# tsai0507/PolishPathPlanning

Hardware: NVIDIA B200
Metric: points/sec kNN(k=16)+normals+slicing (higher is better)
Workload: dtype f32

## Files before the change

polishpathplanning_b200/csrc/api.cu:

```cuda
#include <stdarg.h>
#include <string.h>

#include <algorithm>
#include <cmath>
#include <string>
#include <vector>

#include "ppp_internal.cuh"
#include <cstring>
#include <cuda.h>

static thread_local char g_err[1024] = "";

void ppp_set_error(const char* fmt, ...) {
  va_list ap;
  va_start(ap, fmt);
  vsnprintf(g_err, sizeof(g_err), fmt, ap);
  va_end(ap);
}

#define LOCK(ctx) ApiScope _api_scope(ctx)

#define REQUIRE(cond, msg)            \
  do {                                \
    if (!(cond)) {                    \
      ppp_set_error("%s: %s", __func__, msg); \
      return PPP_ERR_INVALID;         \
    }                                 \
  } while (0)

extern "C" {

int ppp_abi_version(void) { return PPP_ABI_VERSION; }
const char* ppp_last_error(void) { return g_err; }

int ppp_create(int device, ppp_ctx** out) {
  if (!out) { ppp_set_error("ppp_create: out is NULL"); return PPP_ERR_INVALID; }
  *out = nullptr;
  int ndev = 0;
  cudaError_t e = cudaGetDeviceCount(&ndev);
  if (e != cudaSuccess || ndev == 0) {
    ppp_set_error("ppp_create: no CUDA device (%s); libppp_gpu has no CPU fallback",
                  e != cudaSuccess ? cudaGetErrorString(e) : "device count 0");
    cudaGetLastError();
    return PPP_ERR_CUDA;
  }
  if (device < 0 || device >= ndev) { ppp_set_error("ppp_create: device %d out of range [0,%d)", device, ndev); return PPP_ERR_INVALID; }
  PPP_CUDA(cudaSetDevice(device));
  cudaDeviceProp prop;
  PPP_CUDA(cudaGetDeviceProperties(&prop, device));
  if (prop.major < 10) {
    ppp_set_error("ppp_create: device %d is sm_%d%d; this library is built for sm_100a (B200) only", device, prop.major, prop.minor);
    return PPP_ERR_UNSUPPORTED;
  }
  ppp_ctx* ctx = new ppp_ctx();
  ctx->device = device;
  ctx->sm_count = prop.multiProcessorCount;
  ctx->smem_optin = prop.sharedMemPerBlockOptin;
  int prio_lo = 0, prio_hi = 0;
  PPP_CUDA(cudaDeviceGetStreamPriorityRange(&prio_lo, &prio_hi));
  PPP_CUDA(cudaStreamCreateWithPriority(&ctx->main_stream, cudaStreamNonBlocking, prio_lo));
  PPP_CUDA(cudaStreamCreateWithPriority(&ctx->aux_stream, cudaStreamNonBlocking, prio_hi));
  PPP_CUDA(cudaStreamCreateWithFlags(&ctx->copy_stream, cudaStreamNonBlocking));
  PPP_CUDA(cudaHostAlloc(&ctx->fetch_host, FETCH_BYTES + 128, cudaHostAllocMapped));
  *fetch_flag(ctx) = 0u;
  ctx->stream = ctx->main_stream;
  cudaMemPool_t pool;
  PPP_CUDA(cudaDeviceGetDefaultMemPool(&pool, device));
  uint64_t thr = UINT64_MAX;
  PPP_CUDA(cudaMemPoolSetAttribute(pool, cudaMemPoolAttrReleaseThreshold, &thr));
  *out = ctx;
  return PPP_OK;
}

void ppp_destroy(ppp_ctx* ctx) {
  if (!ctx) return;
  cudaSetDevice(ctx->device);
  cudaStreamSynchronize(ctx->main_stream);
  cudaStreamSynchronize(ctx->aux_stream);
  for (auto& kv : ctx->kstats)
    for (auto& p : kv.second.pending) { cudaEventDestroy(p.first); cudaEventDestroy(p.second); }
  for (int t = 0; t < 16; t++)
    for (auto& p : ctx->t_pending[t]) { cudaEventDestroy(p.first); cudaEventDestroy(p.second); }
  cudaStreamDestroy(ctx->main_stream);
  if (ctx->aux_stream) cudaStreamDestroy(ctx->aux_stream);
  if (ctx->copy_stream) cudaStreamDestroy(ctx->copy_stream);
  if (ctx->fetch_host) cudaFreeHost(ctx->fetch_host);
  for (int i = 0; i < 2; i++) if (ctx->scan_state[i]) cudaFree(ctx->scan_state[i]);
  if (ctx->ingest_dev) cudaFree(ctx->ingest_dev);
  delete ctx;
}

void* ppp_stream(ppp_ctx* ctx) { return ctx ? (void*)ctx->main_stream : nullptr; }

int ppp_sync(ppp_ctx* ctx) {
  REQUIRE(ctx, "ctx is NULL");
  PPP_CUDA(cudaStreamSynchronize(ctx->main_stream));
  return PPP_OK;
}

void* ppp_host_alloc(size_t bytes) {
  void* p = nullptr;
  if (cudaMallocHost(&p, bytes ? bytes : 1) != cudaSuccess) { cudaGetLastError(); return nullptr; }
  return p;
}
void ppp_host_free(void* p) { if (p) cudaFreeHost(p); }

int64_t ppp_launch_count(ppp_ctx* ctx) { return ctx ? ctx->launches : 0; }

int ppp_timer_begin(ppp_ctx* ctx, int tag) {
  REQUIRE(ctx && tag >= 0 && tag < 16, "bad ctx/tag");
  LOCK(ctx);
  cudaEvent_t a, b;
  PPP_CUDA(cudaEventCreate(&a));
  PPP_CUDA(cudaEventCreate(&b));
  PPP_CUDA(cudaEventRecord(a, ctx->main_stream));
  ctx->t_pending[tag].emplace_back(a, b);
  return PPP_OK;
}
int ppp_timer_end(ppp_ctx* ctx, int tag) {
  REQUIRE(ctx && tag >= 0 && tag < 16, "bad ctx/tag");
  LOCK(ctx);
  REQUIRE(!ctx->t_pending[tag].empty(), "timer_end without timer_begin");
  PPP_CUDA(cudaEventRecord(ctx->t_pending[tag].back().second, ctx->main_stream));
  return PPP_OK;
}
int ppp_timer_read(ppp_ctx* ctx, int tag, double* total_ms, int64_t* regions, int reset) {
  REQUIRE(ctx && tag >= 0 && tag < 16, "bad ctx/tag");
  LOCK(ctx);
  PPP_CUDA(cudaStreamSynchronize(ctx->main_stream));
  for (auto& p : ctx->t_pending[tag]) {
    float ms = 0;
    PPP_CUDA(cudaEventElapsedTime(&ms, p.first, p.second));
    ctx->t_ms[tag] += ms;
    ctx->t_regions[tag]++;
    cudaEventDestroy(p.first);
    cudaEventDestroy(p.second);
  }
  ctx->t_pending[tag].clear();
  if (total_ms) *total_ms = ctx->t_ms[tag];
  if (regions) *regions = ctx->t_regions[tag];
  if (reset) { ctx->t_ms[tag] = 0; ctx->t_regions[tag] = 0; }
  return PPP_OK;
}

int ppp_kernel_profile(ppp_ctx* ctx, int enable) {
  REQUIRE(ctx, "ctx is NULL");
  LOCK(ctx);
  ctx->profile = enable != 0;
  return PPP_OK;
}
int ppp_kernel_profile_read(ppp_ctx* ctx, char* buf, size_t cap, int reset) {
  REQUIRE(ctx && buf && cap > 0, "bad arguments");
  LOCK(ctx);
  PPP_CUDA(cudaStreamSynchronize(ctx->main_stream));
  PPP_CUDA(cudaStreamSynchronize(ctx->aux_stream));
  std::string s;
  for (auto& kv : ctx->kstats) {
    KernelStat& st = kv.second;
    for (auto& p : st.pending) {
      float ms = 0;
      if (cudaEventElapsedTime(&ms, p.first, p.second) == cudaSuccess) { st.ms += ms; st.launches++; }
      cudaEventDestroy(p.first);
      cudaEventDestroy(p.second);
    }
    st.pending.clear();
    char line[256];
    snprintf(line, sizeof(line), "%s=%.6f:%lld;", kv.first.c_str(), st.ms, (long long)st.launches);
    s += line;
  }
  if (reset) ctx->kstats.clear();
// ... 794 lines not shown
```

polishpathplanning_b200/csrc/grid.cu:

```cuda
#include <stdlib.h>

#include <algorithm>
#include <cmath>

#include "ppp_device.cuh"

namespace {

__device__ __forceinline__ uint32_t f2ord(float f) {
  uint32_t b = __float_as_uint(f);
  return (b & 0x80000000u) ? ~b : (b | 0x80000000u);
}
inline float ord2f(uint32_t u) {
  uint32_t b = (u & 0x80000000u) ? (u & 0x7FFFFFFFu) : ~u;
  float f;
  memcpy(&f, &b, 4);
  return f;
}

__host__ __device__ inline int ds_sub_shift(long long n) {
  int sh = 0;
  while ((n >> sh) >= 16384) sh++;
  return sh;
}
// ... 37 lines not shown
          x[j] = p.x; y[j] = p.y; z[j] = p.z;
        } else {
          const float* p = raw + i * sf;
          x[j] = __ldg(p); y[j] = __ldg(p + 1); z[j] = __ldg(p + 2);
        }
      }
    }
#pragma unroll
    for (int j = 0; j < PPT; j++) {
      int64_t i = base + (int64_t)j * blockDim.x + threadIdx.x;
      if (i >= n) continue;
      bool fin = finite3(x[j], y[j], z[j]);
      const float4 rec = make_float4(x[j], y[j], z[j], fin ? 0.0f : CUDART_NAN_F);
      xyz4[i] = rec;
      PPP_DEV_ASSERT(!sub || (i >> sub_shift) < 16384);
      if (sub && (i & sub_mask) == 0) sub[i >> sub_shift] = rec;
      if (fin) {
        cnt++;
        mn[0] = fminf(mn[0], x[j]); mx[0] = fmaxf(mx[0], x[j]);
        mn[1] = fminf(mn[1], y[j]); mx[1] = fmaxf(mx[1], y[j]);
        mn[2] = fminf(mn[2], z[j]); mx[2] = fmaxf(mx[2], z[j]);
      }
    }
  }
#pragma unroll
  for (int o = 16; o > 0; o >>= 1) {
#pragma unroll
    for (int d = 0; d < 3; d++) {
      mn[d] = fminf(mn[d], __shfl_xor_sync(0xffffffffu, mn[d], o));
      mx[d] = fmaxf(mx[d], __shfl_xor_sync(0xffffffffu, mx[d], o));
    }
    cnt += __shfl_xor_sync(0xffffffffu, cnt, o);
  }
  __shared__ float s_mn[8][3], s_mx[8][3];
  __shared__ unsigned s_cnt[8];
  const int w = threadIdx.x >> 5;
  if ((threadIdx.x & 31) == 0) {
#pragma unroll
    for (int d = 0; d < 3; d++) { s_mn[w][d] = mn[d]; s_mx[w][d] = mx[d]; }
    s_cnt[w] = cnt;
  }
  __syncthreads();
  if (threadIdx.x == 0) {
    unsigned tot = 0;
    for (int i = 0; i < (int)(blockDim.x >> 5); i++) {
      tot += s_cnt[i];
#pragma unroll
      for (int d = 0; d < 3; d++) { mn[d] = fminf(mn[d], s_mn[i][d]); mx[d] = fmaxf(mx[d], s_mx[i][d]); }
    }
    if (tot) {
#pragma unroll
      for (int d = 0; d < 3; d++) {
        atomicMin(&acc->mn[d], f2ord(mn[d]));
        atomicMax(&acc->mx[d], f2ord(mx[d]));
      }
      atomicAdd(&acc->n_finite, (unsigned long long)tot);
    }
  }
}

__device__ __forceinline__ int cell_of(const GridView& g, float x, float y, float z) {
  int cu = clampi(cell_coord_raw(axis_of(x, y, z, g.au), g.min_u, g.inv_h), 0, g.nu - 1);
  int cv = clampi(cell_coord_raw(axis_of(x, y, z, g.av), g.min_v, g.inv_h), 0, g.nv - 1);
  return cv * g.nu + cu;
}

__global__ void __launch_bounds__(256) k_cell_count(GridView g, const float4* __restrict__ xyz4, int64_t n,
                                                    int32_t* __restrict__ counts) {
  pdl_prologue();
  int64_t i = (int64_t)blockIdx.x * blockDim.x + threadIdx.x;
  if (i >= n) return;
  float4 p = __ldg(xyz4 + i);
  if (p.w != p.w) return;
  const int cell = cell_of(g, p.x, p.y, p.z);
  PPP_DEV_ASSERT(cell >= 0 && cell < g.nu * g.nv);
  atomicAdd(counts + cell, 1);
}

__global__ void __launch_bounds__(256) k_cell_scatter(GridView g, const float4* __restrict__ xyz4, int64_t n,
                                                      int32_t* __restrict__ counts, const int32_t* __restrict__ start,
                                                      float4* __restrict__ sorted) {
  pdl_prologue();
  int64_t i = (int64_t)blockIdx.x * blockDim.x + threadIdx.x;
  if (i >= n) return;
  float4 p = __ldg(xyz4 + i);
  if (p.w != p.w) return;
  int c = cell_of(g, p.x, p.y, p.z);
  int slot = __ldg(start + c) + atomicSub(counts + c, 1) - 1;
  PPP_DEV_ASSERT(c >= 0 && c < g.nu * g.nv && slot >= 0 && slot < g.n_sorted);
  sorted[slot] = make_float4(p.x, p.y, p.z, __int_as_float((int)i));
}

__global__ void __launch_bounds__(256) k_extract_order(const float4* __restrict__ sorted, int64_t n, int32_t* __restrict__ order) {
  pdl_prologue();
  int64_t i = (int64_t)blockIdx.x * blockDim.x + threadIdx.x;
  if (i < n) order[i] = __float_as_int(__ldg(&sorted[i].w));
}

constexpr int DS_KTH = 8;
constexpr int DS_THREADS = 512;
__device__ __forceinline__ float ds_ord2f(uint32_t u) {
  uint32_t b = (u & 0x80000000u) ? (u & 0x7FFFFFFFu) : ~u;
  return __uint_as_float(b);
}

__device__ __forceinline__ float ds_kth_smallest(const float* s) {
  float v[2 * DS_THREADS / 32];
#pragma unroll
  for (int i = 0; i < 2 * DS_THREADS / 32; i++) v[i] = s[i * 32 + (threadIdx.x & 31)];
  float kth = CUDART_INF_F;
  for (int r = 0; r < DS_KTH; r++) {
    float mine = CUDART_INF_F;
    int at = 0;
#pragma unroll
    for (int i = 0; i < 2 * DS_THREADS / 32; i++) if (v[i] < mine) { mine = v[i]; at = i; }
    float w = mine;
#pragma unroll
    for (int o = 16; o > 0; o >>= 1) w = fminf(w, __shfl_xor_sync(0xffffffffu, w, o));
    kth = w;
    const unsigned holders = __ballot_sync(0xffffffffu, mine == w && w < CUDART_INF_F);
    if (holders && (int)(threadIdx.x & 31) == __ffs(holders) - 1) {
#pragma unroll
      for (int i = 0; i < 2 * DS_THREADS / 32; i++) if (i == at) v[i] = CUDART_INF_F;
    }
  }
  return kth;
}

struct IngestScratch {
  BBoxAcc acc;
  unsigned ticket;
  unsigned pad[3];
  float samples[2 * 128];
};

__global__ void __launch_bounds__(DS_THREADS) k_density_sample(const float4* __restrict__ xyz4, int64_t n, int64_t stride_s,
                                                               const float4* __restrict__ sub, int m, IngestScratch* __restrict__ scr, int S,
                                                               unsigned* __restrict__ host_out, unsigned* __restrict__ host_flag,
                                                               unsigned seq, const long long* __restrict__ n_dev,
                                                               const unsigned* __restrict__ extra_src, int extra_words) {
  pdl_prologue();
  __shared__ float s_d[2 * DS_THREADS], s_p[2 * DS_THREADS];
  __shared__ bool s_last;
  if (n_dev) {
    n = *n_dev;
    const long long ds_s = n < (long long)gridDim.x ? n : (long long)gridDim.x;
    stride_s = ds_s > 0 ? (n / ds_s > 1 ? n / ds_s : 1) : 1;
    const int sh = ds_sub_shift(n);
    m = (int)((n + ((long long)1 << sh) - 1) >> sh);
  }
  const BBoxAcc* acc = &scr->acc;
  float* out = scr->samples;
  int drop = 2;
  {
    double ext[3];
    for (int d = 0; d < 3; d++) ext[d] = (double)ds_ord2f(acc->mx[d]) - (double)ds_ord2f(acc->mn[d]);
    if (ext[1] < ext[drop]) drop = 1;
    if (ext[0] < ext[drop]) drop = 0;
  }
  const bool has_q = (int64_t)blockIdx.x * stride_s < n;
  const float4 q = has_q ? __ldg(xyz4 + (int64_t)blockIdx.x * stride_s) : make_float4(0.f, 0.f, 0.f, CUDART_NAN_F);
  const bool qfin = q.w == q.w;
  float d0 = CUDART_INF_F, d1 = CUDART_INF_F, p0 = CUDART_INF_F, p1 = CUDART_INF_F;
  if (qfin) {
    constexpr int PPT = 8;
    for (int j0 = (int)threadIdx.x; j0 < m; j0 += DS_THREADS * PPT) {
// ... 151 lines not shown
  for (int d = 0; d < 3; d++) {
    c->bmin[d] = c->n_finite ? ord2f(h.mn[d]) : 3.402823466e+38f;
    c->bmax[d] = c->n_finite ? ord2f(h.mx[d]) : -3.402823466e+38f;
  }
  double ext[3];
  for (int d = 0; d < 3; d++) ext[d] = c->n_finite ? (double)c->bmax[d] - (double)c->bmin[d] : 0.0;
  int drop = 2;
  if (ext[1] < ext[drop]) drop = 1;
  if (ext[0] < ext[drop]) drop = 0;
  c->drop = drop;
  c->au = drop == 0 ? 1 : 0;
  c->av = drop == 2 ? 1 : 2;
  double area = std::max(ext[c->au], 1e-9) * std::max(ext[c->av], 1e-9);
  c->density = c->n_finite > 0 ? (double)c->n_finite / area : 0.0;
  std::vector<float> r2;
  int piled = 0;
  for (int i = 0; i < ds_s; i++)
    if (std::isfinite(ds_h[i]) && ds_h[i] > 0) {
      r2.push_back(ds_h[i]);
      piled += ds_h[DS_SAMPLES + i] * 4.0f < ds_h[i] ? 1 : 0;
    }
  c->mp_state = (r2.size() >= 32 && c->n_finite >= 4096 && piled * 25 > (int)r2.size()) ? 1 : 0;
  if (const char* e = getenv("PPP_PROJECTIONS")) {
    if (e[0] == '1') c->mp_state = 0;
    if (e[0] == '3') c->mp_state = 1;
  }
  if (getenv("PPP_DEBUG"))
    fprintf(stderr, "[ppp] ingest: %d of %zu samples pile up in projection -> %s\n", piled, r2.size(),
            c->mp_state ? "three projections" : "one column grid");
  if (r2.size() >= 16 && c->n_finite >= 64) {
    std::nth_element(r2.begin(), r2.begin() + r2.size() / 2, r2.end());
    const double r2_med = (double)r2[r2.size() / 2];
    const double seen = (double)((c->n + stride_m - 1) / stride_m) * ((double)c->n_finite / (double)c->n);
    const double rho_sub = 7.67 / (3.14159265358979 * r2_med);
    c->density = rho_sub * (double)c->n_finite / std::max(seen, 1.0);
  }
  return PPP_OK;
}

double cloud_cell_for_k(const ppp_cloud* c, int k) {
  if (c->cell_hint > 0) return c->cell_hint;
  double rho = c->density > 0 ? c->density : 1.0;
  double rk = std::sqrt((double)std::max(k, 1) / (3.14159265358979 * rho));
  double f = 1.35;
  if (const char* e = getenv("PPP_CELL_FACTOR")) { double v = atof(e); if (v > 0.5 && v < 4.0) f = v; }
  return f * rk / (double)PPP_KNN_RINGS;
}
double cloud_cell_for_radius(const ppp_cloud* c, double r) {
  (void)c;
  return r * 0.5 * (1.0 + 1e-3);
}

int cloud_get_grid(ppp_cloud* c, double h, GridStore** out) { return cloud_get_grid_drop(c, h, c->drop, out); }

int cloud_get_grid_drop(ppp_cloud* c, double h, int drop, GridStore** out) {
  ppp_ctx* ctx = c->ctx;
  const int au = drop == 0 ? 1 : 0, av = drop == 2 ? 1 : 2;
  double eu = c->n_finite ? (double)c->bmax[au] - (double)c->bmin[au] : 0.0;
  double ev = c->n_finite ? (double)c->bmax[av] - (double)c->bmin[av] : 0.0;
  if (!(h > 0)) h = 1.0;
  while ((std::floor(eu / h) + 2) * (std::floor(ev / h) + 2) > 268435456.0) h *= 1.5;
  for (auto& g : c->grids)
    if (g.drop == drop && std::fabs(g.h - h) <= 1e-9 * h) { *out = &g; return PPP_OK; }
  if (c->grids.size() >= c->grids.capacity()) {
    ppp_set_error("too many different cell sizes on one cloud (%zu grids)", c->grids.size());
    return PPP_ERR_UNSUPPORTED;
  }
  GridStore gs;
  gs.h = h;
  gs.drop = drop;
  GridView& v = gs.v;
  v.au = au; v.av = av;
  v.h = (float)h;
  v.inv_h = 1.0f / v.h;
  v.min_u = c->n_finite ? c->bmin[au] : 0.0f;
  v.min_v = c->n_finite ? c->bmin[av] : 0.0f;
  v.nu = (int)std::floor(eu * (double)v.inv_h) + 2;
  v.nv = (int)std::floor(ev * (double)v.inv_h) + 2;
  v.slack = (float)(h * (double)(v.nu + v.nv) * 9.5367431640625e-07 + 1e-30);
  v.n_sorted = (int)c->n_finite;
  int64_t ncells = (int64_t)v.nu * v.nv;
  PPP_TRY(dev_alloc_keep(ctx, &gs.sorted, (size_t)std::max<int64_t>(c->n_finite, 1) + PPP_SORTED_PAD));
  PPP_TRY(dev_alloc_keep(ctx, &gs.cell_start, (size_t)ncells + 1));
  int32_t* counts = nullptr;
  PPP_TRY(dev_alloc(ctx, &counts, (size_t)ncells));
  PPP_CUDA(cudaMemsetAsync(counts, 0, (size_t)ncells * sizeof(int32_t), ctx->stream));
  v.sorted = gs.sorted;
  v.cell_start = gs.cell_start;
  if (c->n > 0) {
    unsigned blocks = (unsigned)((c->n + 255) / 256);
    PPP_LAUNCH(ctx, "cell_count", k_cell_count, blocks, 256, 0, v, (const float4*)c->xyz4, c->n, counts);
    PPP_CHECK_LAUNCH();
  }
  PPP_TRY(scan_exclusive_i32(ctx, counts, gs.cell_start, ncells));
  if (c->n > 0) {
    unsigned blocks = (unsigned)((c->n + 255) / 256);
    PPP_LAUNCH(ctx, "cell_scatter", k_cell_scatter, blocks, 256, 0, v, (const float4*)c->xyz4, c->n, counts,
               (const int32_t*)gs.cell_start, gs.sorted);
    PPP_CHECK_LAUNCH();
  }
  dev_free(ctx, counts);
  PPP_CUDA(cudaEventCreateWithFlags(&gs.ready, cudaEventDisableTiming));
  PPP_CUDA(cudaEventRecord(gs.ready, ctx->stream));
  c->grids.push_back(gs);
  *out = &c->grids.back();
  return PPP_OK;
}

int cloud_decide_projection(ppp_cloud* c, const GridStore& g) {
  (void)g;
  if (c->mp_state < 0) c->mp_state = 0;
  return PPP_OK;
}

int cloud_get_mp(ppp_cloud* c, double h, int R0, MPSet** out) {
  ppp_ctx* ctx = c->ctx;
  for (auto& m : c->mps)
    if (m.R0 == R0 && std::fabs(m.h - h) <= 1e-9 * h) { *out = &m; return PPP_OK; }
  if (c->mps.size() >= c->mps.capacity()) { ppp_set_error("too many multi-projection index sets on one cloud"); return PPP_ERR_UNSUPPORTED; }
  MPSet m;
  m.h = h; m.R0 = R0;
  for (int p = 0; p < 3; p++) PPP_TRY(cloud_get_grid_drop(c, h, p, &m.g[p]));
  PPP_TRY(dev_alloc_keep(ctx, &m.choice, (size_t)std::max<int64_t>(c->n, 1)));
  unsigned long long* hist = nullptr;
  PPP_TRY(dev_alloc(ctx, &hist, 3));
  PPP_CUDA(cudaMemsetAsync(hist, 0, 3 * sizeof(unsigned long long), ctx->stream));
  if (c->n > 0) {
    G3 G;
    for (int p = 0; p < 3; p++) G.g[p] = m.g[p]->v;
    PPP_LAUNCH(ctx, "mp_choose", k_mp_choose, (unsigned)((c->n + 255) / 256), 256, 0, G, (const float4*)c->xyz4, c->n, R0,
               m.choice, hist);
    PPP_CHECK_LAUNCH();
  }
  if (getenv("PPP_DEBUG")) {
    unsigned long long hh[3] = {0, 0, 0};
    PPP_TRY(fetch_small(ctx, hist, sizeof(hh), hh));
    fprintf(stderr, "[ppp] projections chosen (h = %g, R0 = %d): yz %llu, xz %llu, xy %llu\n", h, R0, hh[0], hh[1], hh[2]);
  }
  dev_free(ctx, hist);
  PPP_CUDA(cudaEventCreateWithFlags(&m.ready, cudaEventDisableTiming));
  PPP_CUDA(cudaEventRecord(m.ready, ctx->stream));
  c->mps.push_back(m);
  *out = &c->mps.back();
  return PPP_OK;
}

int grid_sorted_order(ppp_cloud* c, GridStore& gs) {
  if (gs.order) return PPP_OK;
  ppp_ctx* ctx = c->ctx;
  const int64_t n = gs.v.n_sorted;
  PPP_TRY(dev_alloc_keep(ctx, &gs.order, (size_t)std::max<int64_t>(n, 1)));
  if (n > 0) {
    PPP_LAUNCH(ctx, "extract_order", k_extract_order, (unsigned)((n + 255) / 256), 256, 0, (const float4*)gs.sorted, n, gs.order);
    PPP_CHECK_LAUNCH();
  }
  return PPP_OK;
}

__global__ void k_fetch_small(const unsigned* __restrict__ src, unsigned* __restrict__ dst, int words,
                              unsigned* __restrict__ flag, unsigned seq) {
  pdl_prologue();
  for (int i = threadIdx.x; i < words; i += blockDim.x) dst[i] = src[i];
  __threadfence_system();
  __syncthreads();
  if (threadIdx.x == 0) *(volatile unsigned*)flag = seq;
}

int fetch_wait(ppp_ctx* ctx, unsigned seq) {
  volatile unsigned* flag = fetch_flag(ctx);
  for (unsigned long spin = 1;; spin++) {
    if (*flag == seq) return PPP_OK;
    if ((spin & 0x1FFFul) == 0) {
      cudaError_t e = cudaStreamQuery(ctx->stream);
      if (e == cudaSuccess) {
        if (*flag == seq) return PPP_OK;
        ppp_set_error("fetch: the stream drained without the kernel signalling (sequence %u)", seq);
        return PPP_ERR_CUDA;
      }
      if (e != cudaErrorNotReady) {
        ppp_set_error("fetch: %s", cudaGetErrorString(e));
        return PPP_ERR_CUDA;
      }
    }
  }
// ... 18 lines not shown
```

polishpathplanning_b200/csrc/knn.cu:

```cuda
#include <stdlib.h>

#include <algorithm>
#include <cmath>

#include "ppp_device.cuh"
#include "sortnet.cuh"

namespace {

struct SearchParams {
  GridView g;
  const float4* xyz4;
  const float* q;
  int q_sf;
  int64_t nq;
  int64_t first;
  int cap;
  int kk;
  int mode;
  int R0;
  float r2;
  int32_t* idx_out;
  float* d2_out;
  const int64_t* offsets;
// ... 596 lines not shown
      int a = max(cu - R, 0), b = min(cu + R, g.nu - 1);
      if (a <= b) {
        const int32_t* rowp = g.cell_start + (int64_t)v * g.nu;
        s = __ldg(rowp + a);
        e = __ldg(rowp + b + 1);
      }
    }
    const int n_it = (__reduce_max_sync(0xffffffffu, e - s) + U - 1) / U;
#pragma unroll 1
    for (int it = 0; it < n_it; it++) {
      float4 c4[U];
      bool in[U];
#pragma unroll
      for (int u = 0; u < U; u++) {
        int i = s + it * U + u;
        in[u] = i < e;
        c4[u] = __ldg(g.sorted + (in[u] ? i : 0));
      }
      u64* wptr = store + ns * BD;
#pragma unroll
      for (int u = 0; u < U; u++) {
        float d2 = d2_flann_x2(pack2(qx, qy), qz, c4[u]);
        u64 key = make_key(d2, __float_as_int(c4[u].w));
        if (in[u] && key < tau) {
          *wptr = key;
          wptr += BD;
        }
      }
      ns = (int)(wptr - store) / BD;
      if (ns > C_STORE - U) { overflow = true; tau = 0; }
    }
  }
  if (!valid) return;
  unsigned c[C_SLOTS];
#pragma unroll
  for (int i = 0; i < C_SLOTS; i++) {
    unsigned hi = (unsigned)(store[i * BD] >> 32);
    c[i] = i < ns ? ((hi & 0xFFFFFFE0u) | (unsigned)i) : 0xFFFFFFFFu;
  }
  SortNetU32<C_SLOTS>::sort(c);
  bool ambiguous = false;
#pragma unroll
  for (int i = 0; i + 1 < C_SLOTS; i++) ambiguous |= (i + 1 < ns) && ((c[i] ^ c[i + 1]) < 32u);
  if (overflow || ns > C_SLOTS || ambiguous) {
    int slot = atomicAdd(P.redo_count, 1);
    P.redo_list[slot] = (int32_t)t;
    return;
  }
  float o[4];
  const int m = ns;
  if (!act || m < 3) {
    o[0] = o[1] = o[2] = o[3] = CUDART_NAN_F;
  } else {
    float acc[9] = {0.f, 0.f, 0.f, 0.f, 0.f, 0.f, 0.f, 0.f, 0.f};
    const bool shifted = (P.flags & PPP_COV_SHIFTED) != 0;
    float kx = 0.f, ky = 0.f, kz = 0.f;
    if (shifted) {
      float4 f = __ldg(P.xyz4 + key_idx(store[(c[0] & 31u) * BD]));
      kx = f.x; ky = f.y; kz = f.z;
    }
#pragma unroll
    for (int jb = 0; jb < C_SLOTS; jb += 4) {
      if (jb < m) {
        float4 a[4];
#pragma unroll
        for (int u = 0; u < 4; u++)
          if (jb + u < m) a[u] = __ldg(P.xyz4 + key_idx(store[(c[jb + u] & 31u) * BD]));
#pragma unroll
        for (int u = 0; u < 4; u++) {
          if (jb + u < m) {
            float x = a[u].x, y = a[u].y, z = a[u].z;
            if (shifted) { x = __fsub_rn(x, kx); y = __fsub_rn(y, ky); z = __fsub_rn(z, kz); }
            accumulate_point(acc, x, y, z);
          }
        }
      }
    }
    normal_from_accumulators(acc, m, qx, qy, qz, P.vpx, P.vpy, P.vpz, o);
  }
  store_normal(P.normals, P.nmap, row, P.nsf, o, P.route);
}

__device__ __forceinline__ u64 warp_min_u64(u64 v) {
#pragma unroll
  for (int o = 16; o > 0; o >>= 1) {
    u64 t = __shfl_xor_sync(0xffffffffu, v, o);
    v = t < v ? t : v;
  }
  return v;
}

constexpr int WARPQ_WARPS = 4;

constexpr int WQ_SEG_MAX = 128;

__global__ void __launch_bounds__(WARPQ_WARPS * 32) k_knn_warp(SearchParams P) {
  pdl_prologue();
  extern __shared__ u64 s_keys[];
  __shared__ int s_seg[WARPQ_WARPS][WQ_SEG_MAX];
  __shared__ int s_pre[WARPQ_WARPS][WQ_SEG_MAX + 1];
  const int lane = threadIdx.x & 31, w = threadIdx.x >> 5;
  const GridView& g = P.g;
  const int k = P.cap, kk = P.kk;
  u64* L = s_keys + (size_t)w * 32 * k + lane;
  const int n_redo = *P.redo_count;
  for (int64_t slot = (int64_t)blockIdx.x * WARPQ_WARPS + w; slot < n_redo; slot += (int64_t)gridDim.x * WARPQ_WARPS) {
  const int64_t t = P.redo_list[slot];
  float qx, qy, qz;
  int64_t row;
  if (P.q) {
    const float* qp = P.q + t * P.q_sf;
    qx = __ldg(qp); qy = __ldg(qp + 1); qz = __ldg(qp + 2);
    row = t;
  } else {
    float4 p = __ldg(g.sorted + P.first + t);
    qx = p.x; qy = p.y; qz = p.z;
    row = __float_as_int(p.w);
  }
  const int cu = cell_coord_raw(axis_of(qx, qy, qz, g.au), g.min_u, g.inv_h);
  const int cv = cell_coord_raw(axis_of(qx, qy, qz, g.av), g.min_v, g.inv_h);
  int cnt = 0;
  u64 tau = PPP_KEY_INF;
  u64 mine = PPP_KEY_INF;
  u64 mine2 = PPP_KEY_INF;
  int du = max(max(-cu, cu - (g.nu - 1)), 0), dv0 = max(max(-cv, cv - (g.nv - 1)), 0);
  int R = max(P.R0, max(du, dv0));
  int R_prev = -1;
  while (true) {
    const int v0 = max(cv - R, 0), v1 = min(cv + R, g.nv - 1);
    const int nseg = 2 * (v1 - v0 + 1);
    if (nseg > 0 && nseg <= WQ_SEG_MAX) {
      int* seg_s = s_seg[w];
      int* seg_p = s_pre[w];
      for (int sg0 = 0; sg0 < nseg; sg0 += 32) {
        const int sg = sg0 + lane;
        int s0 = 0, len = 0;
        if (sg < nseg) {
          const int v = v0 + (sg >> 1), part = sg & 1;
          const bool full = abs(v - cv) > R_prev;
          int a, b;
          if (full) { a = max(cu - R, 0); b = part == 0 ? min(cu + R, g.nu - 1) : -1; }
          else if (part == 0) { a = max(cu - R, 0); b = min(cu - R_prev - 1, g.nu - 1); }
          else { a = max(cu + R_prev + 1, 0); b = min(cu + R, g.nu - 1); }
          if (a <= b) {
            const int32_t* rowp = g.cell_start + (int64_t)v * g.nu;
            s0 = __ldg(rowp + a);
            len = __ldg(rowp + b + 1) - s0;
          }
        }
        int inc = len;
#pragma unroll
        for (int o = 1; o < 32; o <<= 1) { int tt = __shfl_up_sync(0xffffffffu, inc, o); if (lane >= o) inc += tt; }
        const int carry = sg0 == 0 ? 0 : seg_p[sg0];
        if (sg < nseg) { seg_s[sg] = s0; seg_p[sg + 1] = carry + inc; }
        if (sg0 == 0 && lane == 0) seg_p[0] = 0;
        __syncwarp();
      }
      const int T = seg_p[nseg];
      for (int base = 0; base < T; base += 128) {
        float4 c4[4];
        bool in[4];
#pragma unroll
        for (int u = 0; u < 4; u++) {
          const int i = base + u * 32 + lane;
          in[u] = i < T;
          int lo = 0, hi = nseg - 1;
          while (lo < hi) { int mid = (lo + hi + 1) >> 1; if (seg_p[mid] <= i) lo = mid; else hi = mid - 1; }
          c4[u] = __ldg(g.sorted + (in[u] ? seg_s[lo] + (i - seg_p[lo]) : 0));
        }
#pragma unroll
        for (int u = 0; u < 4; u++) {
          if (!in[u]) continue;
          u64 key = make_key(d2_flann(qx, qy, qz, c4[u].x, c4[u].y, c4[u].z), __float_as_int(c4[u].w));
          if (key < tau && (cnt < k || key < L[(k - 1) * 32])) list_insert(L, 32, cnt, k, key);
        }
      }
    } else {
    for (int v = v0; v <= v1; v++) {
      const int32_t* rowp = g.cell_start + (int64_t)v * g.nu;
      const bool full = abs(v - cv) > R_prev;
      for (int part = 0; part < (full ? 1 : 2); part++) {
        int a, b;
        if (full) { a = max(cu - R, 0); b = min(cu + R, g.nu - 1); }
        else if (part == 0) { a = max(cu - R, 0); b = min(cu - R_prev - 1, g.nu - 1); }
        else { a = max(cu + R_prev + 1, 0); b = min(cu + R, g.nu - 1); }
        if (a > b) continue;
        const int s = __ldg(rowp + a), e = __ldg(rowp + b + 1);
        for (int i = s + lane; i < e; i += 32) {
          float4 c = __ldg(g.sorted + i);
          u64 key = make_key(d2_flann(qx, qy, qz, c.x, c.y, c.z), __float_as_int(c.w));
          if (key < tau && (cnt < k || key < L[(k - 1) * 32])) list_insert(L, 32, cnt, k, key);
        }
      }
    }
    }
    __syncwarp();
    int head = 0;
    u64 kth = PPP_KEY_INF;
    mine = PPP_KEY_INF;
    mine2 = PPP_KEY_INF;
    for (int j = 0; j < kk; j++) {
      u64 h = head < cnt ? L[head * 32] : PPP_KEY_INF;
      u64 m = warp_min_u64(h);
      if (m == PPP_KEY_INF) break;
      if (h == m) head++;
      if (lane == (j & 31)) { if (j < 32) mine = m; else mine2 = m; }
      kth = (j == kk - 1) ? m : kth;
    }
    if (kth != PPP_KEY_INF && key_d2(kth) < ring_bound2(g, R, cu, cv)) break;
    if (block_covers_grid(g, cu, cv, R)) break;
    if (kth != PPP_KEY_INF) tau = kth;
    R_prev = R;
    R++;
  }
  const int have = __popc(__ballot_sync(0xffffffffu, mine != PPP_KEY_INF)) +
                   __popc(__ballot_sync(0xffffffffu, mine2 != PPP_KEY_INF));
  if (P.idx_out && lane < k) {
    P.idx_out[row * (int64_t)k + lane] = mine != PPP_KEY_INF ? key_idx(mine) : -1;
    if (P.d2_out) P.d2_out[row * (int64_t)k + lane] = mine != PPP_KEY_INF ? key_d2(mine) : CUDART_INF_F;
  }
  if (P.idx_out && 32 + lane < k) {
    P.idx_out[row * (int64_t)k + 32 + lane] = mine2 != PPP_KEY_INF ? key_idx(mine2) : -1;
    if (P.d2_out) P.d2_out[row * (int64_t)k + 32 + lane] = mine2 != PPP_KEY_INF ? key_d2(mine2) : CUDART_INF_F;
  }
  if (P.normals) {
    float o[4];
    if (have < 3) {
      o[0] = o[1] = o[2] = o[3] = CUDART_NAN_F;
    } else {
      float acc[9] = {0.f, 0.f, 0.f, 0.f, 0.f, 0.f, 0.f, 0.f, 0.f};
      const bool shifted = (P.flags & PPP_COV_SHIFTED) != 0;
      float kx = 0.f, ky = 0.f, kz = 0.f;
      float4 rec = make_float4(0.f, 0.f, 0.f, 0.f), rec2 = rec;
      if (mine != PPP_KEY_INF) rec = __ldg(P.xyz4 + key_idx(mine));
      if (mine2 != PPP_KEY_INF) rec2 = __ldg(P.xyz4 + key_idx(mine2));
      for (int j = 0; j < have; j++) {
        const bool lo32 = j < 32;
        float4 a;
        a.x = __shfl_sync(0xffffffffu, lo32 ? rec.x : rec2.x, j & 31);
        a.y = __shfl_sync(0xffffffffu, lo32 ? rec.y : rec2.y, j & 31);
        a.z = __shfl_sync(0xffffffffu, lo32 ? rec.z : rec2.z, j & 31);
        if (shifted && j == 0) { kx = a.x; ky = a.y; kz = a.z; }
        float x = a.x, y = a.y, z = a.z;
        if (shifted) { x = __fsub_rn(x, kx); y = __fsub_rn(y, ky); z = __fsub_rn(z, kz); }
        accumulate_point(acc, x, y, z);
      }
      normal_from_accumulators(acc, have, qx, qy, qz, P.vpx, P.vpy, P.vpz, o);
    }
    if (lane == 0) store_normal(P.normals, P.nmap, row, P.nsf, o, P.route);
  }
  __syncwarp();
  }
}

constexpr int RW_CAPL = 16;

__global__ void __launch_bounds__(WARPQ_WARPS * 32) k_radius_warp(SearchParams P, int32_t* __restrict__ redo2_count,
                                                                  int32_t* __restrict__ redo2_list) {
  pdl_prologue();
  __shared__ u64 s_l[WARPQ_WARPS * 32 * RW_CAPL];
  const int lane = threadIdx.x & 31, w = threadIdx.x >> 5;
  const GridView& g = P.g;
  u64* L = s_l + (size_t)w * 32 * RW_CAPL + lane;
  const int n_redo = *P.redo_count;
  const u64 tau = make_key(P.r2, 0);
  for (int64_t slot = (int64_t)blockIdx.x * WARPQ_WARPS + w; slot < n_redo; slot += (int64_t)gridDim.x * WARPQ_WARPS) {
    const int64_t t = P.redo_list[slot];
    float4 p = __ldg(g.sorted + P.first + t);
    const float qx = p.x, qy = p.y, qz = p.z;
    const int64_t row = __float_as_int(p.w);
    const int cu = cell_coord_raw(axis_of(qx, qy, qz, g.au), g.min_u, g.inv_h);
    const int cv = cell_coord_raw(axis_of(qx, qy, qz, g.av), g.min_v, g.inv_h);
    const int R = P.R0;
    int cnt = 0;
    bool over = false;
    const int v0 = max(cv - R, 0), v1 = min(cv + R, g.nv - 1);
    for (int v = v0; v <= v1; v++) {
      const int32_t* rowp = g.cell_start + (int64_t)v * g.nu;
      int a = max(cu - R, 0), b = min(cu + R, g.nu - 1);
      if (a > b) continue;
      const int s = __ldg(rowp + a), e = __ldg(rowp + b + 1);
      for (int i = s + lane; i < e; i += 32) {
        float4 c = __ldg(g.sorted + i);
        u64 key = make_key(d2_flann(qx, qy, qz, c.x, c.y, c.z), __float_as_int(c.w));
        if (key < tau) {
          if (cnt == RW_CAPL) over = true;
          else list_insert(L, 32, cnt, RW_CAPL, key);
        }
      }
    }
    __syncwarp();
    if (__any_sync(0xffffffffu, over)) {
      if (lane == 0) redo2_list[atomicAdd(redo2_count, 1)] = (int32_t)t;
      continue;
    }
    float acc[9] = {0.f, 0.f, 0.f, 0.f, 0.f, 0.f, 0.f, 0.f, 0.f};
    const bool shifted = (P.flags & PPP_COV_SHIFTED) != 0;
    float kx = 0.f, ky = 0.f, kz = 0.f;
    int head = 0, m = 0;
    while (true) {
      u64 h = head < cnt ? L[head * 32] : PPP_KEY_INF;
      u64 mn = warp_min_u64(h);
      if (mn == PPP_KEY_INF) break;
      if (h == mn) head++;
      float4 a = __ldg(P.xyz4 + key_idx(mn));
      if (shifted && m == 0) { kx = a.x; ky = a.y; kz = a.z; }
      float x = a.x, y = a.y, z = a.z;
      if (shifted) { x = __fsub_rn(x, kx); y = __fsub_rn(y, ky); z = __fsub_rn(z, kz); }
      accumulate_point(acc, x, y, z);
      m++;
    }
    float o[4];
    if (m < 3) o[0] = o[1] = o[2] = o[3] = CUDART_NAN_F;
    else normal_from_accumulators(acc, m, qx, qy, qz, P.vpx, P.vpy, P.vpz, o);
    if (lane == 0) store_normal(P.normals, P.nmap, row, P.nsf, o, P.route);
    __syncwarp();
  }
}

__global__ void __launch_bounds__(128) k_radius_count(SearchParams P, int32_t* __restrict__ counts, int32_t* __restrict__ max_count) {
  pdl_prologue();
  int64_t t = (int64_t)blockIdx.x * blockDim.x + threadIdx.x;
  int cnt = 0;
  bool have = t < P.nq;
  if (P.use_redo) {
    have = t < *P.redo_count;
    if (have) t = P.redo_list[t];
  }
  if (have) {
    const GridView& g = P.g;
    float qx, qy, qz;
    int64_t row;
    if (P.q) {
      const float* qp = P.q + t * P.q_sf;
      qx = __ldg(qp); qy = __ldg(qp + 1); qz = __ldg(qp + 2);
      row = t;
    } else {
      float4 p = __ldg(g.sorted + P.first + t);
      qx = p.x; qy = p.y; qz = p.z;
      row = __float_as_int(p.w);
    }
    const bool mine = P.use_redo || P.choice == nullptr || P.q != nullptr || __ldg(P.choice + row) == P.my_proj;
    if (mine && finite3(qx, qy, qz) && g.n_sorted > 0) {
      int cu = cell_coord_raw(axis_of(qx, qy, qz, g.au), g.min_u, g.inv_h);
      int cv = cell_coord_raw(axis_of(qx, qy, qz, g.av), g.min_v, g.inv_h);
      const float r2 = P.r2;
      visit_annulus(g, cu, cv, -1, P.R0, [&](float4 c) {
        cnt += d2_flann(qx, qy, qz, c.x, c.y, c.z) < r2 ? 1 : 0;
      });
    }
    if (counts && mine) counts[row] = cnt;
  }
  int m = cnt;
#pragma unroll
  for (int o = 16; o > 0; o >>= 1) m = max(m, __shfl_xor_sync(0xffffffffu, m, o));
  if ((threadIdx.x & 31) == 0 && m > 0) atomicMax(max_count, m);
}


__global__ void __launch_bounds__(128) k_principal_curvatures(const int32_t* __restrict__ idx, int64_t nq, int k,
                                                              const float* __restrict__ normals, int nsf,
                                                              float* __restrict__ out, int32_t* __restrict__ nn0) {
  pdl_prologue();
  int64_t t = (int64_t)blockIdx.x * blockDim.x + threadIdx.x;
  if (t >= nq) return;
  const int32_t* nb = idx + t * (int64_t)k;
  float* o = out + 5 * t;
  int m = 0;
  while (m < k && nb[m] >= 0) m++;
  if (m == 0) {
    for (int i = 0; i < 5; i++) o[i] = CUDART_NAN_F;
    if (nn0) nn0[t] = -1;
    return;
  }
  if (nn0) nn0[t] = nb[0];
  const float* n0 = normals + (int64_t)nb[0] * nsf;
  const float a0 = __ldg(n0), a1 = __ldg(n0 + 1), a2 = __ldg(n0 + 2);
  float M[9];
  const float nn[3] = {a0, a1, a2};
#pragma unroll
  for (int i = 0; i < 3; i++)
#pragma unroll
    for (int j = 0; j < 3; j++) M[3 * i + j] = __fsub_rn(i == j ? 1.0f : 0.0f, __fmul_rn(nn[i], nn[j]));
  auto project = [&](int j, float p[3]) {
    const float* nj = normals + (int64_t)nb[j] * nsf;
    const float b0 = __ldg(nj), b1 = __ldg(nj + 1), b2 = __ldg(nj + 2);
#pragma unroll
    for (int i = 0; i < 3; i++)
      p[i] = __fadd_rn(__fmul_rn(M[3 * i], b0), __fadd_rn(__fmul_rn(M[3 * i + 1], b1), __fmul_rn(M[3 * i + 2], b2)));
  };
  float cen[3] = {0.f, 0.f, 0.f};
  for (int j = 0; j < m; j++) {
    float p[3];
    project(j, p);
    cen[0] = __fadd_rn(cen[0], p[0]); cen[1] = __fadd_rn(cen[1], p[1]); cen[2] = __fadd_rn(cen[2], p[2]);
  }
  const float fm = (float)m;
  cen[0] = __fdiv_rn(cen[0], fm); cen[1] = __fdiv_rn(cen[1], fm); cen[2] = __fdiv_rn(cen[2], fm);
  float c00 = 0.f, c01 = 0.f, c02 = 0.f, c11 = 0.f, c12 = 0.f, c22 = 0.f;
  for (int j = 0; j < m; j++) {
// ... 60 lines not shown
    if (ok) {
      const float* row = d2 + i * k;
      double sum = 0.0;
      for (int j = 1; j < k; j++) {
        float v = __ldg(row + j);
        sum = __dadd_rn(sum, sqrt_float ? (double)__fsqrt_rn(v) : __dsqrt_rn((double)v));
      }
      out = (float)__ddiv_rn(sum, (double)(k - 1));
    }
    dist[i] = out;
  }
  unsigned cnt = __syncthreads_count(ok);
  if (threadIdx.x == 0 && cnt) atomicAdd(n_valid, (unsigned long long)cnt);
}

__global__ void k_fill_i32(int32_t* p, int64_t n, int32_t v) {
  pdl_prologue();
  int64_t i = (int64_t)blockIdx.x * blockDim.x + threadIdx.x;
  if (i < n) p[i] = v;
}

__global__ void k_default_rows(const float4* __restrict__ xyz4, int64_t n, int cap, int32_t* idx_out, float* d2_out,
                               float* normals, int nsf, const int32_t* __restrict__ nmap,
                               const NormalRoute* __restrict__ route) {
  pdl_prologue();
  int64_t i = (int64_t)blockIdx.x * blockDim.x + threadIdx.x;
  if (i >= n) return;
  float4 p = __ldg(xyz4 + i);
  if (p.w == p.w) return;
  if (idx_out)
    for (int j = 0; j < cap; j++) {
      idx_out[i * (int64_t)cap + j] = -1;
      if (d2_out) d2_out[i * (int64_t)cap + j] = CUDART_INF_F;
    }
  if (normals) {
    float o[4] = {CUDART_NAN_F, CUDART_NAN_F, CUDART_NAN_F, CUDART_NAN_F};
    store_normal(normals, nmap, i, nsf, o, route);
  }
}

int pick_block(ppp_ctx* ctx, int cap, int* block, size_t* smem) {
  size_t lim = ctx->smem_optin ? ctx->smem_optin : 48 * 1024;
  for (int b = 128; b >= 32; b >>= 1) {
    size_t need = (size_t)cap * 8 * b;
    if (need <= lim) { *block = b; *smem = need; return PPP_OK; }
  }
  ppp_set_error("neighbour list capacity %d exceeds the shared-memory path (max %zu entries per query)", cap,
                lim / (8 * 32));
  return PPP_ERR_UNSUPPORTED;
}

}

int radius_rings(const GridView& g, double r) {
  r *= 1.0 + 1e-6;
  const double Rd = std::ceil((r + (double)g.slack) / (double)g.h - 1e-12);
  if (!(Rd < (double)PPP_RING_MAX)) return PPP_RING_MAX;
  int R = (int)Rd;
  while (R < PPP_RING_MAX && (double)R * (double)g.h - (double)g.slack < r) R++;
  return std::max(R, 0);
}

static int launch_search(ppp_cloud* c, SearchParams& P) {
  ppp_ctx* ctx = c->ctx;
  int block; size_t smem;
  PPP_TRY(pick_block(ctx, std::max(P.cap, 1), &block, &smem));
  if (P.use_redo) {
    block = 32;
    smem = (size_t)std::max(P.cap, 1) * 8 * block;
  }
  if (smem > 40 * 1024)
    PPP_CUDA(cudaFuncSetAttribute(k_search, cudaFuncAttributeMaxDynamicSharedMemorySize, (int)smem));
  if (P.nq > 0) {
    unsigned blocks = (unsigned)((P.nq + block - 1) / block);
    PPP_LAUNCH(ctx, P.use_redo ? "knn_redo" : P.mode == 0 ? (P.normals ? "knn_normals" : "knn") : (P.normals ? "radius_normals" : "radius_fill"),
               k_search, blocks, block, smem, P);
    PPP_CHECK_LAUNCH();
  }
  return PPP_OK;
}

static int prepare_fast(ppp_cloud* c, SearchParams& P, int32_t** redo_out) {
  ppp_ctx* ctx = c->ctx;
  int32_t* redo = nullptr;
  PPP_TRY(dev_alloc(ctx, &redo, (size_t)P.nq + 1));
  PPP_CUDA(cudaMemsetAsync(redo, 0, sizeof(int32_t), ctx->stream));
  P.redo_count = redo;
  P.redo_list = redo + 1;
  P.use_redo = 0;
  *redo_out = redo;
  return PPP_OK;
}

static int launch_knn_fast(ppp_cloud* c, SearchParams& P) {
  ppp_ctx* ctx = c->ctx;
  int32_t* redo = nullptr;
  PPP_TRY(prepare_fast(c, P, &redo));
  constexpr int block = 128;
  const unsigned blocks = (unsigned)((P.nq + block - 1) / block);
  const bool ext = P.q != nullptr;
  auto launch = [&](auto kern, int slots) -> int {
    const size_t smem = (size_t)(slots + 2 * P.R0 + 1) * 4 * block;
    if (smem > 40 * 1024) PPP_CUDA(cudaFuncSetAttribute(kern, cudaFuncAttributeMaxDynamicSharedMemorySize, (int)smem));
    PPP_LAUNCH(ctx, P.normals ? "knn_normals" : "knn", kern, blocks, block, smem, P);
    PPP_CHECK_LAUNCH();
    return PPP_OK;
  };
  if (P.cap <= 16) PPP_TRY(launch(ext ? k_knn16f<128, 8, 7, true> : k_knn16f<128, 8, 7, false>, F_SLOTS));
  else if (P.cap <= 32) PPP_TRY(launch(ext ? k_knnf<32, 16, 6, 128, 6, true> : k_knnf<32, 16, 6, 128, 6, false>, 32 + 16));
  else PPP_TRY(launch(ext ? k_knnf<64, 32, 7, 128, 4, true> : k_knnf<64, 32, 7, 128, 4, false>, 64 + 32));
  {
    P.use_redo = 1;
    size_t smem = (size_t)WARPQ_WARPS * 32 * P.cap * 8;
    if (smem > 40 * 1024) PPP_CUDA(cudaFuncSetAttribute(k_knn_warp, cudaFuncAttributeMaxDynamicSharedMemorySize, (int)smem));
    unsigned blocks = (unsigned)std::min<int64_t>((P.nq + WARPQ_WARPS - 1) / WARPQ_WARPS, (int64_t)ctx->sm_count * 8);
    PPP_LAUNCH(ctx, "knn_redo", k_knn_warp, blocks, WARPQ_WARPS * 32, smem, P);
    PPP_CHECK_LAUNCH();
  }
  if (getenv("PPP_DEBUG")) {
    int32_t n_redo = 0;
    fetch_small(ctx, redo, 4, &n_redo);
    fprintf(stderr, "[ppp] knn fast path: %lld queries, %d handed to the ring-expanding kernel (h=%g, R0=%d)\n",
            (long long)P.nq, n_redo, (double)P.g.h, P.R0);
  }
  dev_free(ctx, redo);
  return PPP_OK;
}

int knn_launch(ppp_cloud* c, const GridStore& gs, const float* q_dev, int64_t nq, int q_stride_f, int64_t first, int k,
               int32_t* idx_dev, float* d2_dev, bool with_normals, const float vp[3], unsigned flags,
               float* normals_dev, int normal_stride_f, const unsigned char* choice, int my_proj) {
  ppp_ctx* ctx = c->ctx;
  SearchParams P{};
  P.g = gs.v; P.xyz4 = c->xyz4; P.q = q_dev; P.q_sf = q_stride_f; P.nq = nq; P.first = first;
  P.cap = k; P.kk = (int)std::min<int64_t>(k, c->n_finite); P.mode = 0; P.R0 = PPP_KNN_RINGS; P.r2 = 0;
  P.idx_out = idx_dev; P.d2_out = d2_dev; P.offsets = nullptr;
  P.normals = with_normals ? normals_dev : nullptr; P.nsf = normal_stride_f; P.nmap = c->nmap; P.route = c->route;
  P.vpx = vp ? vp[0] : 0; P.vpy = vp ? vp[1] : 0; P.vpz = vp ? vp[2] : 0; P.flags = flags;
  P.choice = q_dev ? nullptr : choice; P.my_proj = my_proj;
  if (!q_dev && c->n_finite < c->n && first == 0) {
    unsigned blocks = (unsigned)((c->n + 255) / 256);
    PPP_LAUNCH(ctx, "default_rows", k_default_rows, blocks, 256, 0, (const float4*)c->xyz4, c->n, k, idx_dev, d2_dev,
               P.normals, normal_stride_f, c->nmap, c->route);
    PPP_CHECK_LAUNCH();
  }
  if (k <= 64 && nq > 0) return launch_knn_fast(c, P);
  return launch_search(c, P);
}

int radius_count_launch(ppp_cloud* c, const GridStore& gs, const float* q_dev, int64_t nq, int q_stride_f,
                        int64_t first, float r2, int32_t* counts_dev) {
  ppp_ctx* ctx = c->ctx;
  SearchParams P{};
  P.g = gs.v; P.xyz4 = c->xyz4; P.q = q_dev; P.q_sf = q_stride_f; P.nq = nq; P.first = first;
  P.mode = 1; P.r2 = r2; P.R0 = radius_rings(gs.v, std::sqrt((double)r2));
  int32_t* mx = nullptr;
  PPP_TRY(dev_alloc(ctx, &mx, 1));
  PPP_CUDA(cudaMemsetAsync(mx, 0, 4, ctx->stream));
  if (!q_dev && c->n_finite < c->n && counts_dev) {
    unsigned blocks = (unsigned)((c->n + 255) / 256);
    PPP_LAUNCH(ctx, "fill_i32", k_fill_i32, blocks, 256, 0, counts_dev, c->n, 0);
    PPP_CHECK_LAUNCH();
  }
  if (nq > 0) {
    unsigned blocks = (unsigned)((nq + 127) / 128);
    PPP_LAUNCH(ctx, "radius_count", k_radius_count, blocks, 128, 0, P, counts_dev, mx);
    PPP_CHECK_LAUNCH();
  }
  int hmx = 0;
  PPP_TRY(fetch_small(ctx, mx, 4, &hmx));
  dev_free(ctx, mx);
  return hmx;
}

int radius_fill_launch(ppp_cloud* c, const GridStore& gs, const float* q_dev, int64_t nq, int q_stride_f,
                       int64_t first, float r2, const int64_t* offsets_dev, int32_t* idx_dev, float* d2_dev) {
  int mx = radius_count_launch(c, gs, q_dev, nq, q_stride_f, first, r2, nullptr);
  if (mx < 0) return mx;
  SearchParams P{};
  P.g = gs.v; P.xyz4 = c->xyz4; P.q = q_dev; P.q_sf = q_stride_f; P.nq = nq; P.first = first;
  P.cap = std::max(mx, 1); P.mode = 1; P.r2 = r2; P.R0 = radius_rings(gs.v, std::sqrt((double)r2));
  P.idx_out = idx_dev; P.d2_out = d2_dev; P.offsets = offsets_dev;
  return launch_search(c, P);
}

int normals_radius_launch(ppp_cloud* c, const GridStore& gs, int64_t first, int64_t count, float r2,
                          const float vp[3], unsigned flags, float* normals_dev, int normal_stride_f,
                          const unsigned char* choice, int my_proj) {
  ppp_ctx* ctx = c->ctx;
  SearchParams P{};
  P.g = gs.v; P.xyz4 = c->xyz4; P.q = nullptr; P.nq = count; P.first = first;
  P.mode = 1; P.r2 = r2; P.R0 = radius_rings(gs.v, std::sqrt((double)r2));
  P.normals = normals_dev; P.nsf = normal_stride_f; P.nmap = c->nmap; P.route = c->route;
  P.vpx = vp ? vp[0] : 0; P.vpy = vp ? vp[1] : 0; P.vpz = vp ? vp[2] : 0; P.flags = flags;
  P.choice = choice; P.my_proj = my_proj;
  if (c->n_finite < c->n && first == 0) {
    unsigned blocks = (unsigned)((c->n + 255) / 256);
    PPP_LAUNCH(ctx, "default_rows", k_default_rows, blocks, 256, 0, (const float4*)c->xyz4, c->n, 0, (int32_t*)nullptr,
               (float*)nullptr, normals_dev, normal_stride_f, c->nmap, c->route);
    PPP_CHECK_LAUNCH();
  }
  if (count <= 0) return PPP_OK;
  const double expect = c->density * 3.14159265358979 * (double)r2;
  const bool fast = expect <= 24.0;
  int32_t* redo = nullptr;
  int n_redo = 0;
// ... 94 lines not shown
```

polishpathplanning_b200/csrc/ppp_internal.cuh:

```cuda
#pragma once
#include <cuda_runtime.h>
#include <stdint.h>
#include <stdio.h>

#include <map>
#include <mutex>
#include <string>
#include <vector>

#include "../../include/ppp_gpu.h"

void ppp_set_error(const char* fmt, ...);

#define PPP_CUDA(call)                                                                         \
  do {                                                                                         \
    cudaError_t _e = (call);                                                                   \
    if (_e != cudaSuccess) {                                                                   \
      ppp_set_error("%s:%d: %s -> %s", __FILE__, __LINE__, #call, cudaGetErrorString(_e));      \
      return PPP_ERR_CUDA;                                                                     \
    }                                                                                          \
  } while (0)

#define PPP_TRY(call)              \
  do {                             \
    int _s = (call);               \
    if (_s != PPP_OK) return _s;   \
  } while (0)

struct KernelStat {
  std::vector<std::pair<cudaEvent_t, cudaEvent_t>> pending;
  double ms = 0;
  int64_t launches = 0;
};

struct ppp_ctx {
  int device = 0;
  int sm_count = 148;
  size_t smem_optin = 0;
  cudaStream_t stream = nullptr;
  cudaStream_t main_stream = nullptr;
  cudaStream_t aux_stream = nullptr;
  cudaStream_t copy_stream = nullptr;
  void* fetch_host = nullptr;
  unsigned fetch_seq = 0;
  void* ingest_dev = nullptr;
  bool ingest_clean = false;
  unsigned long long* scan_state[2] = {nullptr, nullptr};
  int64_t scan_state_cap[2] = {0, 0};
  std::vector<void*> temps;
  int api_depth = 0;
  std::recursive_mutex mu;
  int64_t launches = 0;
  bool profile = false;
  bool trace = false;
  cudaEvent_t trace_base = nullptr;
  struct TraceRec { const char* name; int aux; cudaEvent_t a, b; };
  std::vector<TraceRec> trace_recs;
  std::map<std::string, KernelStat> kstats;
  cudaEvent_t t_begin[16] = {}, t_end[16] = {};
  double t_ms[16] = {};
  int64_t t_regions[16] = {};
  std::vector<std::pair<cudaEvent_t, cudaEvent_t>> t_pending[16];
};

struct GridView {
  const float4* sorted;
  const int32_t* cell_start;
  int nu, nv;
  int au, av;
  float min_u, min_v;
  float inv_h, h;
  float slack;
  int n_sorted;
};

constexpr int PPP_MAX_RANKS = 16;
struct NormalRoute {
  int world;
  long long start[PPP_MAX_RANKS + 1];
  float* base[PPP_MAX_RANKS];
};

constexpr int PPP_SORTED_PAD = 160;

constexpr int PPP_KNN_RINGS = 2;

struct GridStore {
  GridView v{};
  int drop = 2;
  float4* sorted = nullptr;
  int32_t* cell_start = nullptr;
  int32_t* order = nullptr;
  double h = 0;
  cudaEvent_t ready = nullptr;
};

struct AuxScope {
  ppp_ctx* ctx;
  cudaStream_t saved;
  bool active;
  AuxScope(ppp_ctx* c, cudaEvent_t after) : ctx(c), saved(c->stream), active(!c->profile) {
    if (!active) return;
    if (after) cudaStreamWaitEvent(ctx->aux_stream, after, 0);
    ctx->stream = ctx->aux_stream;
  }
  ~AuxScope() {
    if (!active) return;
    cudaEvent_t ev;
    if (cudaEventCreateWithFlags(&ev, cudaEventDisableTiming) == cudaSuccess) {
      cudaEventRecord(ev, ctx->aux_stream);
      cudaStreamWaitEvent(ctx->main_stream, ev, 0);
      cudaEventDestroy(ev);
    }
    ctx->stream = saved;
  }
};

struct MPSet {
  double h = 0;
  int R0 = 0;
  GridStore* g[3] = {nullptr, nullptr, nullptr};
  unsigned char* choice = nullptr;
  cudaEvent_t ready = nullptr;
};

struct ppp_cloud {
  ppp_ctx* ctx = nullptr;
  int64_t n = 0;
  int64_t n_finite = 0;
  float4* xyz4 = nullptr;
  float bmin[3] = {0, 0, 0}, bmax[3] = {0, 0, 0};
// ... 183 lines not shown
```

Baseline: 2.319 billion.

## Persist self-cleaning grid count and redo counter buffers to drop per-call memsets

```diff
diff --git a/polishpathplanning_b200/csrc/api.cu b/polishpathplanning_b200/csrc/api.cu
--- a/polishpathplanning_b200/csrc/api.cu
+++ b/polishpathplanning_b200/csrc/api.cu
@@ -86,7 +86,11 @@
   if (ctx->aux_stream) cudaStreamDestroy(ctx->aux_stream);
   if (ctx->copy_stream) cudaStreamDestroy(ctx->copy_stream);
   if (ctx->fetch_host) cudaFreeHost(ctx->fetch_host);
-  for (int i = 0; i < 2; i++) if (ctx->scan_state[i]) cudaFree(ctx->scan_state[i]);
+  for (int i = 0; i < 2; i++) {
+    if (ctx->scan_state[i]) cudaFree(ctx->scan_state[i]);
+    if (ctx->cell_counts[i]) cudaFree(ctx->cell_counts[i]);
+    if (ctx->redo_ctr[i]) cudaFree(ctx->redo_ctr[i]);
+  }
   if (ctx->ingest_dev) cudaFree(ctx->ingest_dev);
   delete ctx;
 }
diff --git a/polishpathplanning_b200/csrc/grid.cu b/polishpathplanning_b200/csrc/grid.cu
--- a/polishpathplanning_b200/csrc/grid.cu
+++ b/polishpathplanning_b200/csrc/grid.cu
@@ -143,6 +143,7 @@
                                                       float4* __restrict__ sorted) {
   pdl_prologue();
   int64_t i = (int64_t)blockIdx.x * blockDim.x + threadIdx.x;
+  PPP_DEV_ASSERT(i != 0 || __ldg(start + (int64_t)g.nu * g.nv) == g.n_sorted);
   if (i >= n) return;
   float4 p = __ldg(xyz4 + i);
   if (p.w != p.w) return;
@@ -460,9 +461,21 @@
   int64_t ncells = (int64_t)v.nu * v.nv;
   PPP_TRY(dev_alloc_keep(ctx, &gs.sorted, (size_t)std::max<int64_t>(c->n_finite, 1) + PPP_SORTED_PAD));
   PPP_TRY(dev_alloc_keep(ctx, &gs.cell_start, (size_t)ncells + 1));
-  int32_t* counts = nullptr;
-  PPP_TRY(dev_alloc(ctx, &counts, (size_t)ncells));
-  PPP_CUDA(cudaMemsetAsync(counts, 0, (size_t)ncells * sizeof(int32_t), ctx->stream));
+  const int si = ctx->stream == ctx->aux_stream ? 1 : 0;
+  if (ctx->cell_counts_cap[si] < ncells || !ctx->cell_counts_clean[si]) {
+    if (ctx->cell_counts_cap[si] < ncells) {
+      if (ctx->cell_counts[si]) PPP_CUDA(cudaFreeAsync(ctx->cell_counts[si], ctx->stream));
+      ctx->cell_counts[si] = nullptr;
+      ctx->cell_counts_cap[si] = 0;
+      const int64_t cap = std::max<int64_t>(ncells + ncells / 4, 4096);
+      PPP_CUDA(cudaMallocAsync((void**)&ctx->cell_counts[si], (size_t)cap * sizeof(int32_t), ctx->stream));
+      ctx->cell_counts_cap[si] = cap;
+    }
+    PPP_CUDA(cudaMemsetAsync(ctx->cell_counts[si], 0, (size_t)ctx->cell_counts_cap[si] * sizeof(int32_t), ctx->stream));
+    ctx->cell_counts_clean[si] = true;
+  }
+  int32_t* counts = ctx->cell_counts[si];
+  ctx->cell_counts_clean[si] = false;
   v.sorted = gs.sorted;
   v.cell_start = gs.cell_start;
   if (c->n > 0) {
@@ -477,7 +490,7 @@
                (const int32_t*)gs.cell_start, gs.sorted);
     PPP_CHECK_LAUNCH();
   }
-  dev_free(ctx, counts);
+  ctx->cell_counts_clean[si] = true;
   PPP_CUDA(cudaEventCreateWithFlags(&gs.ready, cudaEventDisableTiming));
   PPP_CUDA(cudaEventRecord(gs.ready, ctx->stream));
   c->grids.push_back(gs);
diff --git a/polishpathplanning_b200/csrc/knn.cu b/polishpathplanning_b200/csrc/knn.cu
--- a/polishpathplanning_b200/csrc/knn.cu
+++ b/polishpathplanning_b200/csrc/knn.cu
@@ -702,15 +702,24 @@
 }
 
 __device__ __forceinline__ u64 warp_min_u64(u64 v) {
-#pragma unroll
-  for (int o = 16; o > 0; o >>= 1) {
-    u64 t = __shfl_xor_sync(0xffffffffu, v, o);
-    v = t < v ? t : v;
-  }
-  return v;
+  const unsigned hi = __reduce_min_sync(0xffffffffu, (unsigned)(v >> 32));
+  const unsigned lo = __reduce_min_sync(0xffffffffu, (unsigned)(v >> 32) == hi ? (unsigned)v : 0xFFFFFFFFu);
+  return ((u64)hi << 32) | lo;
 }
 
 constexpr int WARPQ_WARPS = 4;
+
+__device__ __forceinline__ void release_redo_counter(const SearchParams& P) {
+  __syncthreads();
+  if (threadIdx.x == 0) {
+    __threadfence();
+    unsigned* ticket = reinterpret_cast<unsigned*>(P.redo_count + 1);
+    if (atomicAdd(ticket, 1u) == gridDim.x - 1) {
+      P.redo_count[0] = 0;
+      *ticket = 0u;
+    }
+  }
+}
 
 constexpr int WQ_SEG_MAX = 128;
 
@@ -871,6 +880,7 @@
   }
   __syncwarp();
   }
+  release_redo_counter(P);
 }
 
 constexpr int RW_CAPL = 16;
@@ -936,6 +946,7 @@
     if (lane == 0) store_normal(P.normals, P.nmap, row, P.nsf, o, P.route);
     __syncwarp();
   }
+  release_redo_counter(P);
 }
 
 __global__ void __launch_bounds__(128) k_radius_count(SearchParams P, int32_t* __restrict__ counts, int32_t* __restrict__ max_count) {
@@ -1162,11 +1173,15 @@
 
 static int prepare_fast(ppp_cloud* c, SearchParams& P, int32_t** redo_out) {
   ppp_ctx* ctx = c->ctx;
+  const int si = ctx->stream == ctx->aux_stream ? 1 : 0;
+  if (!ctx->redo_ctr[si]) {
+    PPP_CUDA(cudaMallocAsync((void**)&ctx->redo_ctr[si], 2 * sizeof(int32_t), ctx->stream));
+    PPP_CUDA(cudaMemsetAsync(ctx->redo_ctr[si], 0, 2 * sizeof(int32_t), ctx->stream));
+  }
   int32_t* redo = nullptr;
-  PPP_TRY(dev_alloc(ctx, &redo, (size_t)P.nq + 1));
-  PPP_CUDA(cudaMemsetAsync(redo, 0, sizeof(int32_t), ctx->stream));
-  P.redo_count = redo;
-  P.redo_list = redo + 1;
+  PPP_TRY(dev_alloc(ctx, &redo, (size_t)std::max<int64_t>(P.nq, 1)));
+  P.redo_count = ctx->redo_ctr[si];
+  P.redo_list = redo;
   P.use_redo = 0;
   *redo_out = redo;
   return PPP_OK;
@@ -1189,6 +1204,12 @@
   if (P.cap <= 16) PPP_TRY(launch(ext ? k_knn16f<128, 8, 7, true> : k_knn16f<128, 8, 7, false>, F_SLOTS));
   else if (P.cap <= 32) PPP_TRY(launch(ext ? k_knnf<32, 16, 6, 128, 6, true> : k_knnf<32, 16, 6, 128, 6, false>, 32 + 16));
   else PPP_TRY(launch(ext ? k_knnf<64, 32, 7, 128, 4, true> : k_knnf<64, 32, 7, 128, 4, false>, 64 + 32));
+  if (getenv("PPP_DEBUG")) {
+    int32_t n_redo = 0;
+    fetch_small(ctx, P.redo_count, 4, &n_redo);
+    fprintf(stderr, "[ppp] knn fast path: %lld queries, %d handed to the ring-expanding kernel (h=%g, R0=%d)\n",
+            (long long)P.nq, n_redo, (double)P.g.h, P.R0);
+  }
   {
     P.use_redo = 1;
     size_t smem = (size_t)WARPQ_WARPS * 32 * P.cap * 8;
@@ -1196,12 +1217,6 @@
     unsigned blocks = (unsigned)std::min<int64_t>((P.nq + WARPQ_WARPS - 1) / WARPQ_WARPS, (int64_t)ctx->sm_count * 8);
     PPP_LAUNCH(ctx, "knn_redo", k_knn_warp, blocks, WARPQ_WARPS * 32, smem, P);
     PPP_CHECK_LAUNCH();
-  }
-  if (getenv("PPP_DEBUG")) {
-    int32_t n_redo = 0;
-    fetch_small(ctx, redo, 4, &n_redo);
-    fprintf(stderr, "[ppp] knn fast path: %lld queries, %d handed to the ring-expanding kernel (h=%g, R0=%d)\n",
-            (long long)P.nq, n_redo, (double)P.g.h, P.R0);
   }
   dev_free(ctx, redo);
   return PPP_OK;
diff --git a/polishpathplanning_b200/csrc/ppp_internal.cuh b/polishpathplanning_b200/csrc/ppp_internal.cuh
--- a/polishpathplanning_b200/csrc/ppp_internal.cuh
+++ b/polishpathplanning_b200/csrc/ppp_internal.cuh
@@ -47,6 +47,10 @@
   bool ingest_clean = false;
   unsigned long long* scan_state[2] = {nullptr, nullptr};
   int64_t scan_state_cap[2] = {0, 0};
+  int32_t* cell_counts[2] = {nullptr, nullptr};
+  int64_t cell_counts_cap[2] = {0, 0};
+  bool cell_counts_clean[2] = {true, true};
+  int32_t* redo_ctr[2] = {nullptr, nullptr};
   std::vector<void*> temps;
   int api_depth = 0;
   std::recursive_mutex mu;
```

After: 2.389 billion, median of 6. +3.0%, better.
